# r9y9/deepvoice3_pytorch

Hardware: NVIDIA H100
Metric: mel-frames/sec training step (B=16,T_mel=800) (higher is better)
Workload: dtype f32 via split 16-bit pairs (fp16 pairs forward, bf16 pairs for gradients; 3 wgmma passes per product, fp32 accumulate)

## Files before the change

### deepvoice3_pytorch_b200/csrc/tc_gemm.cu

```cuda
#include "tc_common.cuh"
#include "../../include/dv3b200.h"

namespace dv3 {

using namespace tc;

constexpr int TC_CONV_THREADS = 512;
constexpr int TC_PRODUCER_REGS = 24;
constexpr int TC_CONSUMER_REGS = 176;
constexpr int TC_EPILOGUE_REGS = 136;
static_assert(TC_PRODUCER_REGS <= 65536 / TC_CONV_THREADS && TC_CONSUMER_REGS >= 65536 / TC_CONV_THREADS &&
              TC_EPILOGUE_REGS >= 65536 / TC_CONV_THREADS, "setmaxnreg direction of each warpgroup");
static_assert(128 * TC_PRODUCER_REGS + 256 * TC_CONSUMER_REGS + 128 * TC_EPILOGUE_REGS <= 65536, "register file");
constexpr int MAX_TAPS_TC = 8;
constexpr int SMEM_LIMIT = 232448;
constexpr int RING_RESERVE = 32768;

template <int STAGE_BYTES, int TILE_COLS, int RESERVE>
struct RingCfg {
    static constexpr int STAGE = STAGE_BYTES;
    static constexpr int NCOLS = TILE_COLS;
    static constexpr int ACC_PITCH = NCOLS + 1;
    static constexpr int ACC_TILE = 128 * ACC_PITCH * 4;
    static constexpr int STAGES_RAW = (SMEM_LIMIT - 2048 - RESERVE - ACC_TILE) / STAGE;
    static constexpr int STAGES = STAGES_RAW > 6 ? 6 : STAGES_RAW;
    static constexpr int SMEM = STAGES * STAGE + ACC_TILE + 1024 + 512;
};

enum { TC_GATED = 0, TC_CONV = 1 };

struct TcMaps { CUtensorMap a[2]; CUtensorMap b[2]; };

struct TcParams {
    int T;
    int Nc;
    int rows_per_tap;
    int k, kb_n;
    int tap_off[MAX_TAPS_TC];
    const float* bias; const float* spk; const float* res;
    float* y; float* save_a; float* save_s;
    int gate_mode, residual;
    float* out; const float* e1; const float* e2; float alpha; int addmode, relu;
    float p_drop; const unsigned long long* seed_ptr; uint32_t salt;
    float gmain;
    int operand_bf16;
};

template <int BK> struct SwizzleOf;
template <> struct SwizzleOf<64> { static constexpr uint32_t layout = WG_SW128, sbo = 1024; };
template <> struct SwizzleOf<32> { static constexpr uint32_t layout = WG_SW64, sbo = 512; };

template <int BK>
__device__ __forceinline__ uint64_t make_desc(uint32_t saddr) {
    return make_wgmma_desc(saddr, 16, SwizzleOf<BK>::sbo, SwizzleOf<BK>::layout);
}

template <int NBOX, int BK, int BR, int NPL = 2>
using TcCfg = RingCfg<NPL * (128 + NBOX * BR) * BK * 2, BR * NBOX, RING_RESERVE>;
static_assert(TcCfg<2, 32, 64>::STAGES == 4, "gated forward: 4-stage ring");
static_assert(TcCfg<1, 32, 128>::STAGES == 4, "128-column conv: 4-stage ring");
static_assert(TcCfg<1, 64, 64>::STAGES == 3, "64-column conv at BK = 64: 3-stage ring");
static_assert(TcCfg<1, 32, 64>::STAGES == 6, "64-column conv at BK = 32: 6-stage ring");
static_assert(TcCfg<2, 64, 64, 1>::STAGES == 4, "single-pass gated forward: 4-stage ring");
static_assert(TcCfg<1, 64, 128, 1>::STAGES == 4, "single-pass 128-column conv at BK = 64: 4-stage ring");
static_assert(TcCfg<1, 32, 128, 1>::STAGES == 6, "single-pass 128-column conv at BK = 32: 6-stage ring");
static_assert(TcCfg<1, 64, 64, 1>::STAGES == 6, "single-pass 64-column conv at BK = 64: 6-stage ring");
static_assert(TcCfg<1, 32, 64, 1>::STAGES == 6, "single-pass 64-column conv at BK = 32: 6-stage ring");

template <int BR>
__device__ __forceinline__ void epilogue_gated(const TcParams& p, const float* arow, uint64_t* acc_empty, int a_row0,
                                               int a_z, int b_row0) {
    const int t = a_row0 + (threadIdx.x & 127), b = a_z, C = p.Nc;
    const bool tv = t < p.T;
    const float* __restrict__ bias = p.bias;
    const float* __restrict__ res = p.res;
    const float* __restrict__ spk = p.spk;
    float* __restrict__ yo = p.y;
    float* __restrict__ ao = p.save_a;
    float* __restrict__ so = p.save_s;
    const bool need_res = (p.gate_mode != 0) || p.residual;
    const size_t base = ((size_t)b * C + b_row0) * p.T + (tv ? t : 0);
#pragma unroll
    for (int c32 = 0; c32 < BR; c32 += 32) {
        float rr[32], sp[32];
        if (tv) {
            const size_t cb = base + (size_t)c32 * p.T;
#pragma unroll
            for (int i = 0; i < 32; ++i) rr[i] = need_res ? __ldg(&res[cb + (size_t)i * p.T]) : 0.f;
            if (spk) {
#pragma unroll
                for (int i = 0; i < 32; ++i) sp[i] = __ldg(&spk[cb + (size_t)i * p.T]);
            }
#pragma unroll
            for (int i = 0; i < 32; ++i) {
                const int c = b_row0 + c32 + i;
                const size_t idx = cb + (size_t)i * p.T;
                float va = arow[c32 + i];
                if (spk) va += sp[i];
                const float a = va + __ldg(&bias[c]);
                const float s = sigmoidf_(arow[BR + c32 + i] + __ldg(&bias[C + c]));
                float y;
                if (p.gate_mode == 0) {
                    y = a * s;
                    if (p.residual) y = (y + rr[i]) * 0.70710678118654752f;
                } else {
                    y = s * a + (1.f - s) * rr[i];
                }
                yo[idx] = y;
                if (ao) ao[idx] = a;
                if (so) so[idx] = s;
            }
        }
        if (c32 + 32 == BR) mbar_arrive(acc_empty);
    }
}

template <int NCOLS>
__device__ __forceinline__ void epilogue_conv(const TcParams& p, const float* arow, uint64_t* acc_empty, int a_row0,
                                              int a_z, int b_row0) {
    const int t = a_row0 + (threadIdx.x & 127), b = a_z;
    const bool tv = t < p.T;
    const DropCfg drop = make_drop(p.p_drop, p.seed_ptr, p.salt);
    const float* __restrict__ bias = p.bias;
    const float* __restrict__ e1 = p.e1;
    const float* __restrict__ e2 = p.e2;
    float* __restrict__ out = p.out;
#pragma unroll 1
    for (int c32 = 0; c32 < NCOLS; c32 += 32) {
        float v[32], x2[32];
        const int n0 = b_row0 + c32;
        const size_t cb = ((size_t)b * p.Nc + n0) * p.T + (tv ? t : 0);
        if (tv) {
#pragma unroll
            for (int i = 0; i < 32; ++i) {
                const bool ok = n0 + i < p.Nc;
                v[i] = (p.addmode != 0 && ok) ? __ldg(&e1[cb + (size_t)i * p.T]) : 0.f;
                x2[i] = (p.addmode == 2 && ok) ? __ldg(&e2[cb + (size_t)i * p.T]) : 0.f;
            }
#pragma unroll
            for (int i = 0; i < 32; ++i) {
                const int n = n0 + i;
                if (n < p.Nc) {
                    const size_t idx = cb + (size_t)i * p.T;
                    float g = arow[c32 + i] * drop_scale(drop, (uint32_t)idx);
                    if (bias) g += __ldg(&bias[n]);
                    if (p.addmode == 1) g += p.alpha * v[i];
                    else if (p.addmode == 2) g += v[i] * (1.f - x2[i]);
                    if (p.relu) g = fmaxf(g, 0.f);
                    out[idx] = g;
                }
            }
        }
        if (c32 + 32 == NCOLS) mbar_arrive(acc_empty);
    }
}

template <class Cfg, int NPL, class Decode, class Load, class Mma, class Gmain, class Epilogue>
__device__ __forceinline__ void tc_pipeline(const TcMaps& maps, int num_units, Decode decode, Load load, Mma mma,
                                            Gmain gmain, Epilogue epilogue) {
    static_assert(NPL == 1 || NPL == 2, "one or two operand planes");
    static_assert(Cfg::NCOLS <= 128, "main + cross accumulators must fit in the registers of a consumer thread");
    static_assert(Cfg::STAGES >= 2, "pipeline needs at least two stages");
    constexpr int STAGE = Cfg::STAGE, STAGES = Cfg::STAGES;
    constexpr int NR = Cfg::NCOLS / 2;
    pdl_trigger();
    extern __shared__ uint8_t smem_raw[];
    uint8_t* smem = reinterpret_cast<uint8_t*>((reinterpret_cast<uintptr_t>(smem_raw) + 1023) & ~(uintptr_t)1023);
    float* acc_tile = reinterpret_cast<float*>(smem + STAGES * STAGE);
    uint64_t* full = reinterpret_cast<uint64_t*>(smem + STAGES * STAGE + Cfg::ACC_TILE);
    uint64_t* empty = full + STAGES;
    uint64_t* acc_full = empty + STAGES;
    uint64_t* acc_empty = acc_full + 1;
    const int warp = threadIdx.x >> 5, lane = threadIdx.x & 31;

    if (threadIdx.x == 0) {
#pragma unroll
        for (int pl = 0; pl < NPL; ++pl) prefetch_tmap(&maps.a[pl]);
#pragma unroll
        for (int pl = 0; pl < NPL; ++pl) prefetch_tmap(&maps.b[pl]);
        for (int s = 0; s < STAGES; ++s) { mbar_init(&full[s], 1); mbar_init(&empty[s], 2); }
        mbar_init(acc_full, 256);
        mbar_init(acc_empty, 128);
        fence_barrier_init();
    }
    __syncthreads();
    pdl_wait();

    if (warp >= 12) {
        setmaxnreg_inc<TC_EPILOGUE_REGS>();
        int n = 0;
        for (int u = blockIdx.x; u < num_units; u += gridDim.x, ++n) {
            const auto w = decode(u);
            mbar_wait(acc_full, n & 1);
            epilogue(w, acc_tile, acc_empty);
        }
    } else if (warp >= 8) {
        setmaxnreg_dec<TC_PRODUCER_REGS>();
        if (warp == 8 && lane == 0) {
            int it = 0;
            for (int u = blockIdx.x; u < num_units; u += gridDim.x) {
                const auto w = decode(u);
                for (int kit = 0; kit < w.n_iters; ++kit, ++it) {
                    const int s = it % STAGES, ph = (it / STAGES) & 1;
                    mbar_wait(&empty[s], ph ^ 1);
                    mbar_arrive_expect_tx(&full[s], STAGE);
                    load(w, kit, smem + s * STAGE, &full[s]);
                }
            }
        }
    } else {
        setmaxnreg_inc<TC_CONSUMER_REGS>();
        const int wg = warp >> 2, wq = warp & 3;
        float acc[NR], xacc[NPL == 2 ? NR : 1];
        int it = 0, n = 0;
        for (int u = blockIdx.x; u < num_units; u += gridDim.x, ++n) {
            const auto w = decode(u);
#pragma unroll
            for (int i = 0; i < NR; ++i) {
                acc[i] = 0.f;
                if constexpr (NPL == 2) xacc[i] = 0.f;
            }
            for (int kit = 0; kit < w.n_iters; ++kit, ++it) {
                const int s = it % STAGES, ph = (it / STAGES) & 1;
                mbar_wait(&full[s], ph);
                wgmma_fence();
                mma(smem + s * STAGE, wg, acc, xacc);
                wgmma_commit();
                wgmma_wait<1>();
                if (kit > 0 && (threadIdx.x & 127) == 0) mbar_arrive(&empty[(it - 1) % STAGES]);
            }
            wgmma_wait<0>();
            if (w.n_iters > 0 && (threadIdx.x & 127) == 0) mbar_arrive(&empty[(it - 1) % STAGES]);
            const float gm = gmain(w);
            mbar_wait(acc_empty, (n & 1) ^ 1);
#pragma unroll
            for (int i = 0; i < NR; ++i) {
                float* dst = &acc_tile[(64 * wg + frag_row(i, wq, lane)) * Cfg::ACC_PITCH + frag_col(i, lane)];
                if constexpr (NPL == 2) *dst = fmaf(xacc[i], LO_INV, acc[i] * gm);
                else *dst = acc[i] * gm;
            }
            mbar_arrive(acc_full);
        }
    }
}

template <int MODE, int NBOX, int BR, int BK, bool BF16, int NPL>
__global__ void __launch_bounds__(TC_CONV_THREADS, 1)
tc_conv_kernel(const __grid_constant__ TcMaps maps, const __grid_constant__ TcParams p, int tiles_x, int tiles_y,
               int num_tiles) {
    using Cfg = TcCfg<NBOX, BK, BR, NPL>;
    constexpr int NCOLS = Cfg::NCOLS;
    constexpr int TILE = 128 * BK * 2, TILE_B = BR * BK * 2;
    constexpr int B_OFF = NPL * TILE;
    constexpr int A_HALF = 64 * BK * 2;
    const int n_iters = p.k * p.kb_n;

    struct Tile { int a_row0, a_z, b_row0, b_row1, n_iters; };
    auto decode = [&](int tile) {
        Tile w;
        const int ty = tile % tiles_y, r = tile / tiles_y;
        w.a_z = r / tiles_x;
        w.a_row0 = (r % tiles_x) * 128;
        if (MODE == TC_GATED) { w.b_row0 = ty * BR; w.b_row1 = p.Nc + ty * BR; }
        else { w.b_row0 = ty * BR * NBOX; w.b_row1 = w.b_row0 + BR; }
        w.n_iters = n_iters;
        return w;
    };
    auto load = [&](const Tile& w, int kit, uint8_t* st, uint64_t* bar) {
        const int j = kit / p.kb_n, kb = kit - j * p.kb_n;
        const int ax = kb * BK, ay = w.a_row0 + p.tap_off[j];
        const int by0 = j * p.rows_per_tap + w.b_row0, by1 = j * p.rows_per_tap + w.b_row1;
#pragma unroll
        for (int pl = 0; pl < NPL; ++pl) {
            tma_load_3d(st + pl * TILE, &maps.a[pl], bar, ax, ay, w.a_z);
            uint8_t* bdst = st + B_OFF + pl * NBOX * TILE_B;
            tma_load_3d(bdst, &maps.b[pl], bar, ax, by0, 0);
            if (NBOX == 2) tma_load_3d(bdst + TILE_B, &maps.b[pl], bar, ax, by1, 0);
        }
    };
    auto mma = [&](const uint8_t* st, int wg, float* acc, float* xacc) {
        const uint32_t sa = smem_u32(st) + wg * A_HALF, sb = smem_u32(st + B_OFF);
#pragma unroll
        for (int kk = 0; kk < BK / 16; ++kk) {
            const uint32_t ko = kk * 32;
            const uint64_t a0 = make_desc<BK>(sa + ko), b0 = make_desc<BK>(sb + ko);
            wgmma_mma<NCOLS, 0, 0>(BF16, acc, a0, b0, 1);
            if constexpr (NPL == 2) {
                const uint64_t a1 = make_desc<BK>(sa + TILE + ko), b1 = make_desc<BK>(sb + NBOX * TILE_B + ko);
                wgmma_mma<NCOLS, 0, 0>(BF16, xacc, a0, b1, 1);
                wgmma_mma<NCOLS, 0, 0>(BF16, xacc, a1, b0, 1);
            }
        }
    };
    auto gmain = [&](const Tile&) { return p.gmain; };
    auto epilogue = [&](const Tile& w, const float* acc_tile, uint64_t* acc_empty) {
        const float* arow = acc_tile + (threadIdx.x & 127) * Cfg::ACC_PITCH;
        if (MODE == TC_GATED) epilogue_gated<BR>(p, arow, acc_empty, w.a_row0, w.a_z, w.b_row0);
        else epilogue_conv<NCOLS>(p, arow, acc_empty, w.a_row0, w.a_z, w.b_row0);
    };
    tc_pipeline<Cfg, NPL>(maps, num_tiles, decode, load, mma, gmain, epilogue);
}

struct TcMnParams {
    int T, B, Mw, Nw, k;
    int tap_off[MAX_TAPS_TC];
    int nsplit, batches_per_split, kb_n;
    int tiles_n, tiles_m, num_units;
    float* dw; long long split_stride;
    int msplit; long long s_m, s_mh, s_n, s_j;
    float gcoef;
};

constexpr int WG_BOX = 64 * 32 * 2;
template <int NPL>
using WgCfg = RingCfg<NPL * 4 * WG_BOX, 128, 0>;
static_assert(WgCfg<2>::STAGES == 5, "two-plane weight gradient: 5-stage ring");
static_assert(WgCfg<1>::STAGES == 6, "single-pass weight gradient: 6-stage ring");
static_assert(WgCfg<2>::SMEM <= SMEM_LIMIT && WgCfg<1>::SMEM <= SMEM_LIMIT, "weight gradient shared memory");

template <int NPL>
__global__ void __launch_bounds__(TC_CONV_THREADS, 1)
tc_wgrad_mn_kernel(const __grid_constant__ TcMaps maps, const __grid_constant__ TcMnParams p) {
    using Cfg = WgCfg<NPL>;
    constexpr int A_PL = 2 * WG_BOX, B_PL = 2 * WG_BOX;
    constexpr uint32_t LBO = 4096, SBO = 1024;

    struct Unit { int m0, n0, j, s, b_beg, n_iters; };
    auto decode = [&](int u) {
        Unit w;
        w.n0 = (u % p.tiles_n) * 128;
        int r = u / p.tiles_n;
        w.m0 = (r % p.tiles_m) * 128;
        r /= p.tiles_m;
        w.j = r % p.k;
        w.s = r / p.k;
        w.b_beg = w.s * p.batches_per_split;
        const int b_end = min(p.B, w.b_beg + p.batches_per_split);
        w.n_iters = (b_end > w.b_beg ? b_end - w.b_beg : 0) * p.kb_n;
        return w;
    };
    auto load = [&](const Unit& w, int kit, uint8_t* st, uint64_t* bar) {
        const int bi = kit / p.kb_n, tc_ = kit - bi * p.kb_n;
        const int b = w.b_beg + bi, t0 = tc_ * 32;
#pragma unroll
        for (int pl = 0; pl < NPL; ++pl) {
#pragma unroll
            for (int h = 0; h < 2; ++h)
                tma_load_3d(st + pl * A_PL + h * WG_BOX, &maps.a[pl], bar, w.m0 + h * 64, t0, b);
#pragma unroll
            for (int q = 0; q < 2; ++q)
                tma_load_3d(st + NPL * A_PL + pl * B_PL + q * WG_BOX, &maps.b[pl], bar, w.n0 + q * 64,
                            t0 + p.tap_off[w.j], b);
        }
    };
    auto mma = [&](const uint8_t* st, int wg, float* acc, float* xacc) {
        const uint32_t sa = smem_u32(st);
#pragma unroll
        for (int kk = 0; kk < 2; ++kk) {
            const uint32_t ko = kk * 16 * 128;
            const uint64_t a0 = make_wgmma_desc(sa + wg * WG_BOX + ko, LBO, SBO, WG_SW128);
            const uint64_t b0 = make_wgmma_desc(sa + NPL * A_PL + ko, LBO, SBO, WG_SW128);
            wgmma_mma<128, 1, 1>(true, acc, a0, b0, 1);
            if constexpr (NPL == 2) {
                const uint64_t a1 = make_wgmma_desc(sa + A_PL + wg * WG_BOX + ko, LBO, SBO, WG_SW128);
                const uint64_t b1 = make_wgmma_desc(sa + 2 * A_PL + B_PL + ko, LBO, SBO, WG_SW128);
                wgmma_mma<128, 1, 1>(true, xacc, a0, b1, 1);
                wgmma_mma<128, 1, 1>(true, xacc, a1, b0, 1);
            }
        }
    };
    auto gmain = [&](const Unit& w) { return 1.f + p.gcoef * (float)(2 * w.n_iters); };
    auto epilogue = [&](const Unit& w, const float* acc_tile, uint64_t* acc_empty) {
        const int r = threadIdx.x & 127;
        float* __restrict__ out = p.dw + (size_t)w.s * p.split_stride + (size_t)w.j * p.s_j;
        const int rows = min(128, p.Mw - w.m0), cols = min(128, p.Nw - w.n0);
        if (p.s_n == 1) {
            if (r < cols) {
                float* __restrict__ o = out + w.n0 + r;
#pragma unroll 4
                for (int i = 0; i < rows; ++i) {
                    const int m = w.m0 + i;
                    o[(size_t)(m % p.msplit) * p.s_m + (size_t)(m / p.msplit) * p.s_mh] = acc_tile[i * Cfg::ACC_PITCH + r];
                }
            }
        } else if (r < rows) {
            const int m = w.m0 + r;
            float* __restrict__ o = out + (size_t)(m % p.msplit) * p.s_m + (size_t)(m / p.msplit) * p.s_mh +
                                    (size_t)w.n0 * p.s_n;
            const float* arow = acc_tile + r * Cfg::ACC_PITCH;
#pragma unroll 4
            for (int c = 0; c < cols; ++c) o[(size_t)c * p.s_n] = arow[c];
        }
        mbar_arrive(acc_empty);
    };
    tc_pipeline<Cfg, NPL>(maps, p.num_units, decode, load, mma, gmain, epilogue);
}

typedef CUresult (*EncodeTiledFn)(CUtensorMap*, CUtensorMapDataType, cuuint32_t, void*, const cuuint64_t*,
                                  const cuuint64_t*, const cuuint32_t*, const cuuint32_t*, CUtensorMapInterleave,
                                  CUtensorMapSwizzle, CUtensorMapL2promotion, CUtensorMapFloatOOBfill);

static EncodeTiledFn encode_fn() {
    static const EncodeTiledFn fn = [] {
        void* f = nullptr;
        cudaDriverEntryPointQueryResult qres;
        cudaError_t e = cudaGetDriverEntryPoint("cuTensorMapEncodeTiled", &f, cudaEnableDefault, &qres);
        return (e == cudaSuccess) ? (EncodeTiledFn)f : (EncodeTiledFn) nullptr;
    }();
    return fn;
}

int encode_tmap_bf16_3d(CUtensorMap* map, const void* base, uint64_t d0, uint64_t d1, uint64_t d2,
                        uint64_t stride1_bytes, uint64_t stride2_bytes, uint32_t box0, uint32_t box1) {
    const EncodeTiledFn enc = encode_fn();
    if (!enc) { set_error("cuTensorMapEncodeTiled entry point unavailable"); return 1; }
    cuuint64_t dims[3] = {d0, d1, d2};
    cuuint64_t strides[2] = {stride1_bytes, stride2_bytes};
    cuuint32_t box[3] = {box0, box1, 1};
    cuuint32_t estr[3] = {1, 1, 1};
    const CUtensorMapSwizzle sw = box0 * 2 == 128 ? CU_TENSOR_MAP_SWIZZLE_128B : CU_TENSOR_MAP_SWIZZLE_64B;
    CUresult r = enc(map, CU_TENSOR_MAP_DATA_TYPE_BFLOAT16, 3, const_cast<void*>(base), dims, strides, box, estr,
                     CU_TENSOR_MAP_INTERLEAVE_NONE, sw, CU_TENSOR_MAP_L2_PROMOTION_L2_256B,
                     CU_TENSOR_MAP_FLOAT_OOB_FILL_NONE);
    if (r != CUDA_SUCCESS) {
        set_error("cuTensorMapEncodeTiled failed (%d): dims=(%llu,%llu,%llu) strides=(%llu,%llu) box=(%u,%u)", (int)r,
                  (unsigned long long)d0, (unsigned long long)d1, (unsigned long long)d2,
                  (unsigned long long)stride1_bytes, (unsigned long long)stride2_bytes, box0, box1);
        return 1;
    }
    return 0;
}

template <typename K>
static int ensure_smem(K kern, int bytes, const char* what) {
    cudaError_t e = cudaFuncSetAttribute(kern, cudaFuncAttributeMaxDynamicSharedMemorySize, bytes);
    if (e != cudaSuccess) { set_error("%s: cannot set %d B dynamic smem: %s", what, bytes, cudaGetErrorString(e)); return 1; }
    return 0;
}

template <class Cfg, auto kern, typename... Args>
static int launch_persistent(int units, cudaStream_t st, const char* what, const Args&... args) {
    static const int configured = ensure_smem(kern, Cfg::SMEM, what);
    if (configured) return 1;
    const int sms = config().sms, grid = units < sms ? units : sms;
    cudaError_t e = launch_k(kern, dim3(grid), dim3(TC_CONV_THREADS), (size_t)Cfg::SMEM, st, args...);
    if (e != cudaSuccess) { set_error("%s: launch failed: %s", what, cudaGetErrorString(e)); return 1; }
    return check_launch(what);
}

template <int MODE, int NBOX, int BR, int BK, bool BF16, int NPL>
static int launch_conv_fmt(const TcMaps& maps, const TcParams& p, int tiles_x, int tiles_y, int batch, cudaStream_t st,
                           const char* what) {
    const int num_tiles = tiles_x * tiles_y * batch;
    return launch_persistent<TcCfg<NBOX, BK, BR, NPL>, tc_conv_kernel<MODE, NBOX, BR, BK, BF16, NPL>>(
        num_tiles, st, what, maps, p, tiles_x, tiles_y, num_tiles);
}

template <int MODE, int NBOX, int BR, int BK, int NPL = 2>
static int launch_conv(const TcMaps& maps, const TcParams& p, int tiles_x, int tiles_y, int batch, cudaStream_t st,
                       const char* what) {
    if (p.operand_bf16)
        return launch_conv_fmt<MODE, NBOX, BR, BK, true, NPL>(maps, p, tiles_x, tiles_y, batch, st, what);
    return launch_conv_fmt<MODE, NBOX, BR, BK, false, NPL>(maps, p, tiles_x, tiles_y, batch, st, what);
}

static void fill_taps_tc(int* tap_off, int k, int dilation, int causal, bool transpose) {
    const int padl = causal ? (k - 1) * dilation : (k - 1) / 2 * dilation;
    for (int j = 0; j < MAX_TAPS_TC; ++j)
        tap_off[j] = j < k ? (transpose ? (padl - j * dilation) : (j * dilation - padl)) : 0;
}

static inline const void* plane(const void* base, int pl, long long plane_elems) {
    return (const char*)base + (size_t)pl * plane_elems * 2;
}

}

using namespace dv3;

extern "C" {

int dv3_tc_supported(int B, int C, int T, int k) {
    return (C % 128 == 0) && T >= 1 && k >= 1 && k <= MAX_TAPS_TC && B >= 1 && B <= 65535;
}
int dv3_tc_conv_supported(int B, int Cin, int Cout, int T, int k) {
    return T >= 1 && k >= 1 && k <= MAX_TAPS_TC && B >= 1 && B <= 65535 && (k == 1 || Cout % 128 == 0) && Cin >= 8 &&
           Cout >= 1;
}

int dv3_tc_convblock_fwd(const void* xd, const void* w, int npl, const float* bias, const float* spk,
                         const float* res, float* y, float* save_a, float* save_s, int B, int C, int T, int k,
                         int dilation, int causal, int mode, int residual, const void* fuse, void* stream) {
    DV3_REQUIRE(dv3_tc_supported(B, C, T, k), "tc_convblock_fwd: unsupported shape B=%d C=%d T=%d k=%d", B, C, T, k);
    DV3_REQUIRE(npl == 1 || npl == 2, "tc_convblock_fwd: npl must be 1 or 2");
    DV3_REQUIRE(fuse == nullptr, "tc_convblock_fwd: fuse must be NULL");
    TcMaps maps;
    const int t_tiles = (T + 127) / 128;
    const int BK = npl == 2 ? 32 : 64;
    for (int pl = 0; pl < npl; ++pl) {
        if (encode_tmap_bf16_3d(&maps.a[pl], plane(xd, pl, (long long)B * T * C), C, T, B, (uint64_t)C * 2,
                                (uint64_t)T * C * 2, BK, 128)) return 1;
        if (encode_tmap_bf16_3d(&maps.b[pl], plane(w, pl, (long long)k * 2 * C * C), C, (uint64_t)k * 2 * C, 1,
                                (uint64_t)C * 2, (uint64_t)k * 2 * C * C * 2, BK, 64)) return 1;
    }
    TcParams p = {};
    p.T = T; p.Nc = C; p.rows_per_tap = 2 * C; p.k = k; p.kb_n = C / BK;
    fill_taps_tc(p.tap_off, k, dilation, causal, false);
    p.bias = bias; p.spk = spk; p.res = res; p.y = y; p.save_a = save_a; p.save_s = save_s;
    p.gate_mode = mode; p.residual = residual;
    p.gmain = 1.f + config().tc_gamma * (float)(p.k * p.kb_n * (BK / 16));
    cudaStream_t st = (cudaStream_t)stream;
    if (npl == 1)
        return launch_conv_fmt<TC_GATED, 2, 64, 64, false, 1>(maps, p, t_tiles, C / 64, B, st, "tc_convblock_fwd");
    return launch_conv_fmt<TC_GATED, 2, 64, 32, false, 2>(maps, p, t_tiles, C / 64, B, st, "tc_convblock_fwd");
}

int dv3_tc_conv(const void* a, const void* w, int npl, float* out, int B, int Kc, int Nc, int T, int k, int dilation,
                int causal, int transpose_taps, const float* bias, int relu, float p_drop,
                const unsigned long long* seed_ptr, unsigned salt, int addmode, const float* e1, const float* e2,
                float alpha, const void* fuse, void* stream) {
    DV3_REQUIRE(k >= 1 && k <= MAX_TAPS_TC && (k == 1 || Nc % 128 == 0) && B <= 65535,
                "tc_conv: unsupported shape B=%d Kc=%d Nc=%d T=%d k=%d", B, Kc, Nc, T, k);
    DV3_REQUIRE(npl == 1 || npl == 2, "tc_conv: npl must be 1 or 2");
    DV3_REQUIRE(fuse == nullptr, "tc_conv: fuse must be NULL");
    const int Kp = (Kc + 7) / 8 * 8;
    const int t_tiles = (T + 127) / 128;
    cudaStream_t st = (cudaStream_t)stream;
    const long long tiles128 = (long long)t_tiles * ((Nc + 127) / 128) * B;
    const bool narrow = Nc > 64 && (k == 1 || Nc % 64 == 0) && tiles128 < 100;
    const bool k64 = Kc % 64 == 0;
    const int bk = ((narrow || npl == 1) && k64) ? 64 : 32, br = narrow ? 64 : 128;
    TcMaps maps;
    for (int pl = 0; pl < npl; ++pl) {
        if (encode_tmap_bf16_3d(&maps.a[pl], plane(a, pl, (long long)B * T * Kp), Kc, T, B, (uint64_t)Kp * 2,
                                (uint64_t)T * Kp * 2, bk, 128)) return 1;
        if (encode_tmap_bf16_3d(&maps.b[pl], plane(w, pl, (long long)k * Nc * Kp), Kc, (uint64_t)k * Nc, 1,
                                (uint64_t)Kp * 2, (uint64_t)k * Nc * Kp * 2, bk, br)) return 1;
    }
    TcParams p = {};
    p.T = T; p.Nc = Nc; p.rows_per_tap = Nc; p.k = k; p.kb_n = (Kc + bk - 1) / bk;
    fill_taps_tc(p.tap_off, k, dilation, causal, transpose_taps != 0);
    p.out = out; p.bias = bias; p.relu = relu; p.e1 = e1; p.e2 = e2; p.alpha = alpha; p.addmode = addmode;
    p.p_drop = p_drop; p.seed_ptr = seed_ptr; p.salt = salt;
    p.gmain = 1.f + config().tc_gamma * (float)(p.k * p.kb_n * (bk / 16));
    p.operand_bf16 = transpose_taps ? 1 : 0;
    const int tiles_y = (Nc + br - 1) / br;
    if (npl == 1) {
        if (narrow) {
            if (k64) return launch_conv<TC_CONV, 1, 64, 64, 1>(maps, p, t_tiles, tiles_y, B, st, "tc_conv(64)");
            return launch_conv<TC_CONV, 1, 64, 32, 1>(maps, p, t_tiles, tiles_y, B, st, "tc_conv(64,bk32)");
        }
        if (k64) return launch_conv<TC_CONV, 1, 128, 64, 1>(maps, p, t_tiles, tiles_y, B, st, "tc_conv(128,bk64)");
        return launch_conv<TC_CONV, 1, 128, 32, 1>(maps, p, t_tiles, tiles_y, B, st, "tc_conv(128)");
    }
    if (narrow) {
        if (k64) return launch_conv<TC_CONV, 1, 64, 64>(maps, p, t_tiles, tiles_y, B, st, "tc_conv(64)");
        return launch_conv<TC_CONV, 1, 64, 32>(maps, p, t_tiles, tiles_y, B, st, "tc_conv(64,bk32)");
    }
    return launch_conv<TC_CONV, 1, 128, 32>(maps, p, t_tiles, tiles_y, B, st, "tc_conv(128)");
}

constexpr double WG_UNIT_ITERS = 25.0;
constexpr double WG_SLAB_BYTES_PER_ITER = 1.5e6;
int dv3_tc_wgrad_nsplit(int B, int Mw, int Nw, int T, int k) {
    const long long tk = (long long)((Mw + 127) / 128) * ((Nw + 127) / 128) * k;
    const long long kb_n = (T + 31) / 32, sms = config().sms;
    const double slab = (double)Mw * Nw * k * 8.0 / WG_SLAB_BYTES_PER_ITER;
    auto cost = [&](int ns) {
        const long long bps = (B + ns - 1) / ns, U = tk * ns, U_full = tk * (ns - 1), G = U < sms ? U : sms;
        const long long L = bps * kb_n, L_last = (B - (ns - 1) * bps) * kb_n;
        return (double)((U_full + G - 1) / G) * (double)(L - L_last) +
               (double)((U + G - 1) / G) * ((double)L_last + WG_UNIT_ITERS) + ns * slab;
    };
    double best = 0.0;
    for (int bps = B, prev = 0; bps >= 1; --bps) {
        const int ns = (B + bps - 1) / bps;
        if (ns != prev && (prev == 0 || cost(ns) < best)) best = cost(ns);
        prev = ns;
    }
    for (int bps = B, prev = 0; bps >= 1; --bps) {
        const int ns = (B + bps - 1) / bps;
        if (ns != prev && cost(ns) <= 1.03 * best) return ns;
        prev = ns;
    }
    return 1;
}

int dv3_tc_wgrad_mn_npl(const void* dy, const void* xd, int npl, float* dw_partials, long long split_stride, int B,
                        int Mw, int Nw, int T, int k, int dilation, int causal, int msplit, long long s_m,
                        long long s_mh, long long s_n, long long s_j, void* stream) {
    DV3_REQUIRE(k >= 1 && k <= MAX_TAPS_TC && B <= 65535, "tc_wgrad_mn: unsupported shape k=%d", k);
    DV3_REQUIRE(npl == 1 || npl == 2, "tc_wgrad_mn: npl must be 1 or 2");
    const int Mp = (Mw + 7) / 8 * 8, Np = (Nw + 7) / 8 * 8;
    TcMaps maps;
    for (int pl = 0; pl < npl; ++pl) {
        if (encode_tmap_bf16_3d(&maps.a[pl], plane(dy, pl, (long long)B * T * Mp), Mw, T, B, (uint64_t)Mp * 2,
                                (uint64_t)T * Mp * 2, 64, 32)) return 1;
        if (encode_tmap_bf16_3d(&maps.b[pl], plane(xd, pl, (long long)B * T * Np), Nw, T, B, (uint64_t)Np * 2,
                                (uint64_t)T * Np * 2, 64, 32)) return 1;
    }
    TcMnParams p = {};
    p.T = T; p.B = B; p.Mw = Mw; p.Nw = Nw; p.k = k; p.kb_n = (T + 31) / 32;
    fill_taps_tc(p.tap_off, k, dilation, causal, false);
    p.nsplit = dv3_tc_wgrad_nsplit(B, Mw, Nw, T, k);
    p.batches_per_split = (B + p.nsplit - 1) / p.nsplit;
    p.tiles_n = (Nw + 127) / 128; p.tiles_m = (Mw + 127) / 128;
    const long long units = (long long)p.tiles_n * p.tiles_m * k * p.nsplit;
    DV3_REQUIRE(units < (1ll << 31), "tc_wgrad_mn: %lld work units", units);
    p.num_units = (int)units;
    p.dw = dw_partials; p.split_stride = split_stride;
    p.msplit = msplit; p.s_m = s_m; p.s_mh = s_mh; p.s_n = s_n; p.s_j = s_j;
    p.gcoef = config().tc_gamma;
    cudaStream_t st = (cudaStream_t)stream;
    if (npl == 1)
        return launch_persistent<WgCfg<1>, tc_wgrad_mn_kernel<1>>(p.num_units, st, "tc_wgrad_mn", maps, p);
    return launch_persistent<WgCfg<2>, tc_wgrad_mn_kernel<2>>(p.num_units, st, "tc_wgrad_mn", maps, p);
}

int dv3_tc_wgrad_mn(const void* dy, const void* xd, float* dw_partials, long long split_stride, int B, int Mw,
                    int Nw, int T, int k, int dilation, int causal, int msplit, long long s_m, long long s_mh,
                    long long s_n, long long s_j, void* stream) {
    return dv3_tc_wgrad_mn_npl(dy, xd, 2, dw_partials, split_stride, B, Mw, Nw, T, k, dilation, causal, msplit, s_m,
                               s_mh, s_n, s_j, stream);
}

}
```

Baseline: 1.545 million.

## Load one shared activation window per K-block and reuse it across conv taps

For two-plane bf16 transposed-tap convolutions (the backward data gradient), the kernel now loads a single activation window covering all tap offsets once per K block into a double-buffered shared-memory slot. Each tap's wgmma reads that window at a shifted row offset instead of issuing a separate 128-row TMA load per tap. The loop order changes to kb-major with taps inner, and new mbarriers manage the window slots. The aim is to cut redundant global and L2 traffic for activations when k>1. In exchange the weight ring is capped at 4 stages to make room, and the window slots add synchronization.

```diff
diff --git a/deepvoice3_pytorch_b200/csrc/tc_gemm.cu b/deepvoice3_pytorch_b200/csrc/tc_gemm.cu
--- a/deepvoice3_pytorch_b200/csrc/tc_gemm.cu
+++ b/deepvoice3_pytorch_b200/csrc/tc_gemm.cu
@@ -1,3 +1,4 @@
+#include <type_traits>
 #include "tc_common.cuh"
 #include "../../include/dv3b200.h"
 
@@ -15,16 +16,19 @@
 constexpr int MAX_TAPS_TC = 8;
 constexpr int SMEM_LIMIT = 232448;
 constexpr int RING_RESERVE = 32768;
-
-template <int STAGE_BYTES, int TILE_COLS, int RESERVE>
+constexpr int WIN_ROWS_MAX = 256;
+
+template <int STAGE_BYTES, int TILE_COLS, int RESERVE, int WIN_SLOT = 0, int WIN_SLOTS = 0, int MAX_STAGES = 6>
 struct RingCfg {
     static constexpr int STAGE = STAGE_BYTES;
+    static constexpr int WSLOT = WIN_SLOT, WSLOTS = WIN_SLOTS;
+    static constexpr int WIN = WSLOT * WSLOTS;
     static constexpr int NCOLS = TILE_COLS;
     static constexpr int ACC_PITCH = NCOLS + 1;
     static constexpr int ACC_TILE = 128 * ACC_PITCH * 4;
-    static constexpr int STAGES_RAW = (SMEM_LIMIT - 2048 - RESERVE - ACC_TILE) / STAGE;
-    static constexpr int STAGES = STAGES_RAW > 6 ? 6 : STAGES_RAW;
-    static constexpr int SMEM = STAGES * STAGE + ACC_TILE + 1024 + 512;
+    static constexpr int STAGES_RAW = (SMEM_LIMIT - 2048 - RESERVE - WIN - ACC_TILE) / STAGE;
+    static constexpr int STAGES = STAGES_RAW > MAX_STAGES ? MAX_STAGES : STAGES_RAW;
+    static constexpr int SMEM = WIN + STAGES * STAGE + ACC_TILE + 1024 + 512;
 };
 
 enum { TC_GATED = 0, TC_CONV = 1 };
@@ -37,6 +41,8 @@
     int rows_per_tap;
     int k, kb_n;
     int tap_off[MAX_TAPS_TC];
+    int win_off, win_rows;
+    int win_shift[MAX_TAPS_TC];
     const float* bias; const float* spk; const float* res;
     float* y; float* save_a; float* save_s;
     int gate_mode, residual;
@@ -66,6 +72,12 @@
 static_assert(TcCfg<1, 32, 128, 1>::STAGES == 6, "single-pass 128-column conv at BK = 32: 6-stage ring");
 static_assert(TcCfg<1, 64, 64, 1>::STAGES == 6, "single-pass 64-column conv at BK = 64: 6-stage ring");
 static_assert(TcCfg<1, 32, 64, 1>::STAGES == 6, "single-pass 64-column conv at BK = 32: 6-stage ring");
+
+template <int NBOX, int BK, int BR, int NPL = 2>
+using TcWinCfg = RingCfg<NPL * NBOX * BR * BK * 2, BR * NBOX, 0, NPL * WIN_ROWS_MAX * BK * 2, 2, 4>;
+static_assert(TcWinCfg<1, 32, 128>::STAGES == 4 && TcWinCfg<1, 64, 64>::STAGES == 4 && TcWinCfg<1, 32, 64>::STAGES == 4,
+              "window path: 4-stage weight rings");
+static_assert(TcWinCfg<1, 64, 64>::SMEM <= SMEM_LIMIT, "window path shared memory");
 
 template <int BR>
 __device__ __forceinline__ void epilogue_gated(const TcParams& p, const float* arow, uint64_t* acc_empty, int a_row0,
@@ -155,22 +167,27 @@
     }
 }
 
-template <class Cfg, int NPL, class Decode, class Load, class Mma, class Gmain, class Epilogue>
+struct NoWindow {};
+template <class Cfg, int NPL, class Decode, class Load, class Mma, class Gmain, class Epilogue, class LoadWin = NoWindow>
 __device__ __forceinline__ void tc_pipeline(const TcMaps& maps, int num_units, Decode decode, Load load, Mma mma,
-                                            Gmain gmain, Epilogue epilogue) {
+                                            Gmain gmain, Epilogue epilogue, int taps = 1, uint32_t win_bytes = 0,
+                                            LoadWin load_win = {}) {
     static_assert(NPL == 1 || NPL == 2, "one or two operand planes");
     static_assert(Cfg::NCOLS <= 128, "main + cross accumulators must fit in the registers of a consumer thread");
     static_assert(Cfg::STAGES >= 2, "pipeline needs at least two stages");
-    constexpr int STAGE = Cfg::STAGE, STAGES = Cfg::STAGES;
+    constexpr int STAGE = Cfg::STAGE, STAGES = Cfg::STAGES, WSLOTS = Cfg::WSLOTS;
     constexpr int NR = Cfg::NCOLS / 2;
     pdl_trigger();
     extern __shared__ uint8_t smem_raw[];
-    uint8_t* smem = reinterpret_cast<uint8_t*>((reinterpret_cast<uintptr_t>(smem_raw) + 1023) & ~(uintptr_t)1023);
+    uint8_t* const wins = reinterpret_cast<uint8_t*>((reinterpret_cast<uintptr_t>(smem_raw) + 1023) & ~(uintptr_t)1023);
+    uint8_t* const smem = wins + Cfg::WIN;
     float* acc_tile = reinterpret_cast<float*>(smem + STAGES * STAGE);
     uint64_t* full = reinterpret_cast<uint64_t*>(smem + STAGES * STAGE + Cfg::ACC_TILE);
     uint64_t* empty = full + STAGES;
     uint64_t* acc_full = empty + STAGES;
     uint64_t* acc_empty = acc_full + 1;
+    uint64_t* wfull = acc_empty + 1;
+    uint64_t* wempty = wfull + WSLOTS;
     const int warp = threadIdx.x >> 5, lane = threadIdx.x & 31;
 
     if (threadIdx.x == 0) {
@@ -181,6 +198,7 @@
         for (int s = 0; s < STAGES; ++s) { mbar_init(&full[s], 1); mbar_init(&empty[s], 2); }
         mbar_init(acc_full, 256);
         mbar_init(acc_empty, 128);
+        for (int s = 0; s < WSLOTS; ++s) { mbar_init(&wfull[s], 1); mbar_init(&wempty[s], 2); }
         fence_barrier_init();
     }
     __syncthreads();
@@ -197,10 +215,20 @@
     } else if (warp >= 8) {
         setmaxnreg_dec<TC_PRODUCER_REGS>();
         if (warp == 8 && lane == 0) {
-            int it = 0;
+            int it = 0, wit = 0;
             for (int u = blockIdx.x; u < num_units; u += gridDim.x) {
                 const auto w = decode(u);
-                for (int kit = 0; kit < w.n_iters; ++kit, ++it) {
+                for (int kit = 0, j = 0; kit < w.n_iters; ++kit, ++it) {
+                    if constexpr (WSLOTS > 0) {
+                        if (j == 0) {
+                            const int ws = wit % WSLOTS;
+                            mbar_wait(&wempty[ws], ((wit / WSLOTS) & 1) ^ 1);
+                            mbar_arrive_expect_tx(&wfull[ws], win_bytes);
+                            load_win(w, kit, wins + ws * Cfg::WSLOT, &wfull[ws]);
+                            ++wit;
+                        }
+                        if (++j == taps) j = 0;
+                    }
                     const int s = it % STAGES, ph = (it / STAGES) & 1;
                     mbar_wait(&empty[s], ph ^ 1);
                     mbar_arrive_expect_tx(&full[s], STAGE);
@@ -212,7 +240,7 @@
         setmaxnreg_inc<TC_CONSUMER_REGS>();
         const int wg = warp >> 2, wq = warp & 3;
         float acc[NR], xacc[NPL == 2 ? NR : 1];
-        int it = 0, n = 0;
+        int it = 0, wit = 0, n = 0;
         for (int u = blockIdx.x; u < num_units; u += gridDim.x, ++n) {
             const auto w = decode(u);
 #pragma unroll
@@ -220,17 +248,28 @@
                 acc[i] = 0.f;
                 if constexpr (NPL == 2) xacc[i] = 0.f;
             }
-            for (int kit = 0; kit < w.n_iters; ++kit, ++it) {
+            for (int kit = 0, j = 0; kit < w.n_iters; ++kit, ++it) {
                 const int s = it % STAGES, ph = (it / STAGES) & 1;
+                if constexpr (WSLOTS > 0) {
+                    if (j == 0) mbar_wait(&wfull[wit % WSLOTS], (wit / WSLOTS) & 1);
+                }
                 mbar_wait(&full[s], ph);
                 wgmma_fence();
-                mma(smem + s * STAGE, wg, acc, xacc);
+                if constexpr (WSLOTS > 0) mma(smem + s * STAGE, wins + (wit % WSLOTS) * Cfg::WSLOT, j, wg, acc, xacc);
+                else mma(smem + s * STAGE, wg, acc, xacc);
                 wgmma_commit();
                 wgmma_wait<1>();
                 if (kit > 0 && (threadIdx.x & 127) == 0) mbar_arrive(&empty[(it - 1) % STAGES]);
+                if constexpr (WSLOTS > 0) {
+                    if (kit > 0 && j == 0 && (threadIdx.x & 127) == 0) mbar_arrive(&wempty[(wit + WSLOTS - 1) % WSLOTS]);
+                    if (++j == taps) { j = 0; ++wit; }
+                }
             }
             wgmma_wait<0>();
-            if (w.n_iters > 0 && (threadIdx.x & 127) == 0) mbar_arrive(&empty[(it - 1) % STAGES]);
+            if (w.n_iters > 0 && (threadIdx.x & 127) == 0) {
+                mbar_arrive(&empty[(it - 1) % STAGES]);
+                if constexpr (WSLOTS > 0) mbar_arrive(&wempty[(wit + WSLOTS - 1) % WSLOTS]);
+            }
             const float gm = gmain(w);
             mbar_wait(acc_empty, (n & 1) ^ 1);
 #pragma unroll
@@ -244,15 +283,15 @@
     }
 }
 
-template <int MODE, int NBOX, int BR, int BK, bool BF16, int NPL>
-__global__ void __launch_bounds__(TC_CONV_THREADS, 1)
-tc_conv_kernel(const __grid_constant__ TcMaps maps, const __grid_constant__ TcParams p, int tiles_x, int tiles_y,
-               int num_tiles) {
-    using Cfg = TcCfg<NBOX, BK, BR, NPL>;
+template <int MODE, int NBOX, int BR, int BK, bool BF16, int NPL, bool WIN>
+__device__ __forceinline__ void tc_conv_body(const TcMaps& maps, const TcParams& p, int tiles_x, int tiles_y,
+                                             int num_tiles) {
+    using Cfg = std::conditional_t<WIN, TcWinCfg<NBOX, BK, BR, NPL>, TcCfg<NBOX, BK, BR, NPL>>;
     constexpr int NCOLS = Cfg::NCOLS;
     constexpr int TILE = 128 * BK * 2, TILE_B = BR * BK * 2;
-    constexpr int B_OFF = NPL * TILE;
+    constexpr int B_OFF = WIN ? 0 : NPL * TILE;
     constexpr int A_HALF = 64 * BK * 2;
+    constexpr int ROW = BK * 2, WPLANE = WIN_ROWS_MAX * ROW;
     const int n_iters = p.k * p.kb_n;
 
     struct Tile { int a_row0, a_z, b_row0, b_row1, n_iters; };
@@ -267,12 +306,14 @@
         return w;
     };
     auto load = [&](const Tile& w, int kit, uint8_t* st, uint64_t* bar) {
-        const int j = kit / p.kb_n, kb = kit - j * p.kb_n;
+        int j, kb;
+        if constexpr (WIN) { kb = kit / p.k; j = kit - kb * p.k; }
+        else { j = kit / p.kb_n; kb = kit - j * p.kb_n; }
         const int ax = kb * BK, ay = w.a_row0 + p.tap_off[j];
         const int by0 = j * p.rows_per_tap + w.b_row0, by1 = j * p.rows_per_tap + w.b_row1;
 #pragma unroll
         for (int pl = 0; pl < NPL; ++pl) {
-            tma_load_3d(st + pl * TILE, &maps.a[pl], bar, ax, ay, w.a_z);
+            if constexpr (!WIN) tma_load_3d(st + pl * TILE, &maps.a[pl], bar, ax, ay, w.a_z);
             uint8_t* bdst = st + B_OFF + pl * NBOX * TILE_B;
             tma_load_3d(bdst, &maps.b[pl], bar, ax, by0, 0);
             if (NBOX == 2) tma_load_3d(bdst + TILE_B, &maps.b[pl], bar, ax, by1, 0);
@@ -292,13 +333,50 @@
             }
         }
     };
+    auto load_win = [&](const Tile& w, int kit, uint8_t* slot, uint64_t* bar) {
+        const int ax = kit / p.k * BK, ay = w.a_row0 + p.win_off;
+#pragma unroll
+        for (int pl = 0; pl < NPL; ++pl) tma_load_3d(slot + pl * WPLANE, &maps.a[pl], bar, ax, ay, w.a_z);
+    };
+    auto mma_win = [&](const uint8_t* st, const uint8_t* slot, int j, int wg, float* acc, float* xacc) {
+        const uint32_t sa = smem_u32(slot) + (64 * wg + p.win_shift[j]) * ROW, sb = smem_u32(st);
+#pragma unroll
+        for (int kk = 0; kk < BK / 16; ++kk) {
+            const uint32_t ko = kk * 32;
+            const uint64_t a0 = make_desc<BK>(sa + ko), b0 = make_desc<BK>(sb + ko);
+            wgmma_mma<NCOLS, 0, 0>(BF16, acc, a0, b0, 1);
+            if constexpr (NPL == 2) {
+                const uint64_t a1 = make_desc<BK>(sa + WPLANE + ko), b1 = make_desc<BK>(sb + NBOX * TILE_B + ko);
+                wgmma_mma<NCOLS, 0, 0>(BF16, xacc, a0, b1, 1);
+                wgmma_mma<NCOLS, 0, 0>(BF16, xacc, a1, b0, 1);
+            }
+        }
+    };
     auto gmain = [&](const Tile&) { return p.gmain; };
     auto epilogue = [&](const Tile& w, const float* acc_tile, uint64_t* acc_empty) {
         const float* arow = acc_tile + (threadIdx.x & 127) * Cfg::ACC_PITCH;
         if (MODE == TC_GATED) epilogue_gated<BR>(p, arow, acc_empty, w.a_row0, w.a_z, w.b_row0);
         else epilogue_conv<NCOLS>(p, arow, acc_empty, w.a_row0, w.a_z, w.b_row0);
     };
-    tc_pipeline<Cfg, NPL>(maps, num_tiles, decode, load, mma, gmain, epilogue);
+    if constexpr (WIN)
+        tc_pipeline<Cfg, NPL>(maps, num_tiles, decode, load, mma_win, gmain, epilogue, p.k,
+                              (uint32_t)(NPL * p.win_rows * ROW), load_win);
+    else
+        tc_pipeline<Cfg, NPL>(maps, num_tiles, decode, load, mma, gmain, epilogue);
+}
+
+template <int MODE, int NBOX, int BR, int BK, bool BF16, int NPL>
+__global__ void __launch_bounds__(TC_CONV_THREADS, 1)
+tc_conv_kernel(const __grid_constant__ TcMaps maps, const __grid_constant__ TcParams p, int tiles_x, int tiles_y,
+               int num_tiles) {
+    tc_conv_body<MODE, NBOX, BR, BK, BF16, NPL, false>(maps, p, tiles_x, tiles_y, num_tiles);
+}
+
+template <int MODE, int NBOX, int BR, int BK, bool BF16, int NPL>
+__global__ void __launch_bounds__(TC_CONV_THREADS, 1)
+tc_conv_window_kernel(const __grid_constant__ TcMaps maps, const __grid_constant__ TcParams p, int tiles_x,
+                      int tiles_y, int num_tiles) {
+    tc_conv_body<MODE, NBOX, BR, BK, BF16, NPL, true>(maps, p, tiles_x, tiles_y, num_tiles);
 }
 
 struct TcMnParams {
@@ -452,6 +530,11 @@
 static int launch_conv_fmt(const TcMaps& maps, const TcParams& p, int tiles_x, int tiles_y, int batch, cudaStream_t st,
                            const char* what) {
     const int num_tiles = tiles_x * tiles_y * batch;
+    if constexpr (MODE == TC_CONV && BF16 && NPL == 2) {
+        if (p.win_rows > 0)
+            return launch_persistent<TcWinCfg<NBOX, BK, BR, NPL>, tc_conv_window_kernel<MODE, NBOX, BR, BK, BF16, NPL>>(
+                num_tiles, st, what, maps, p, tiles_x, tiles_y, num_tiles);
+    }
     return launch_persistent<TcCfg<NBOX, BK, BR, NPL>, tc_conv_kernel<MODE, NBOX, BR, BK, BF16, NPL>>(
         num_tiles, st, what, maps, p, tiles_x, tiles_y, num_tiles);
 }
@@ -468,6 +551,17 @@
     const int padl = causal ? (k - 1) * dilation : (k - 1) / 2 * dilation;
     for (int j = 0; j < MAX_TAPS_TC; ++j)
         tap_off[j] = j < k ? (transpose ? (padl - j * dilation) : (j * dilation - padl)) : 0;
+}
+
+static int set_window(TcParams& p) {
+    int lo = p.tap_off[0], hi = p.tap_off[0];
+    for (int j = 1; j < p.k; ++j) { lo = min(lo, p.tap_off[j]); hi = max(hi, p.tap_off[j]); }
+    p.win_rows = 0;
+    if (p.k == 1 || 128 + hi - lo > WIN_ROWS_MAX) return 128;
+    p.win_off = lo;
+    p.win_rows = 128 + hi - lo;
+    for (int j = 0; j < p.k; ++j) p.win_shift[j] = p.tap_off[j] - lo;
+    return p.win_rows;
 }
 
 static inline const void* plane(const void* base, int pl, long long plane_elems) {
@@ -497,15 +591,15 @@
     TcMaps maps;
     const int t_tiles = (T + 127) / 128;
     const int BK = npl == 2 ? 32 : 64;
+    TcParams p = {};
+    p.T = T; p.Nc = C; p.rows_per_tap = 2 * C; p.k = k; p.kb_n = C / BK;
+    fill_taps_tc(p.tap_off, k, dilation, causal, false);
     for (int pl = 0; pl < npl; ++pl) {
         if (encode_tmap_bf16_3d(&maps.a[pl], plane(xd, pl, (long long)B * T * C), C, T, B, (uint64_t)C * 2,
                                 (uint64_t)T * C * 2, BK, 128)) return 1;
         if (encode_tmap_bf16_3d(&maps.b[pl], plane(w, pl, (long long)k * 2 * C * C), C, (uint64_t)k * 2 * C, 1,
                                 (uint64_t)C * 2, (uint64_t)k * 2 * C * C * 2, BK, 64)) return 1;
     }
-    TcParams p = {};
-    p.T = T; p.Nc = C; p.rows_per_tap = 2 * C; p.k = k; p.kb_n = C / BK;
-    fill_taps_tc(p.tap_off, k, dilation, causal, false);
     p.bias = bias; p.spk = spk; p.res = res; p.y = y; p.save_a = save_a; p.save_s = save_s;
     p.gate_mode = mode; p.residual = residual;
     p.gmain = 1.f + config().tc_gamma * (float)(p.k * p.kb_n * (BK / 16));
@@ -530,16 +624,17 @@
     const bool narrow = Nc > 64 && (k == 1 || Nc % 64 == 0) && tiles128 < 100;
     const bool k64 = Kc % 64 == 0;
     const int bk = ((narrow || npl == 1) && k64) ? 64 : 32, br = narrow ? 64 : 128;
+    TcParams p = {};
+    p.T = T; p.Nc = Nc; p.rows_per_tap = Nc; p.k = k; p.kb_n = (Kc + bk - 1) / bk;
+    fill_taps_tc(p.tap_off, k, dilation, causal, transpose_taps != 0);
+    const int a_rows = (transpose_taps && npl == 2) ? set_window(p) : 128;
     TcMaps maps;
     for (int pl = 0; pl < npl; ++pl) {
         if (encode_tmap_bf16_3d(&maps.a[pl], plane(a, pl, (long long)B * T * Kp), Kc, T, B, (uint64_t)Kp * 2,
-                                (uint64_t)T * Kp * 2, bk, 128)) return 1;
+                                (uint64_t)T * Kp * 2, bk, a_rows)) return 1;
         if (encode_tmap_bf16_3d(&maps.b[pl], plane(w, pl, (long long)k * Nc * Kp), Kc, (uint64_t)k * Nc, 1,
                                 (uint64_t)Kp * 2, (uint64_t)k * Nc * Kp * 2, bk, br)) return 1;
     }
-    TcParams p = {};
-    p.T = T; p.Nc = Nc; p.rows_per_tap = Nc; p.k = k; p.kb_n = (Kc + bk - 1) / bk;
-    fill_taps_tc(p.tap_off, k, dilation, causal, transpose_taps != 0);
     p.out = out; p.bias = bias; p.relu = relu; p.e1 = e1; p.e2 = e2; p.alpha = alpha; p.addmode = addmode;
     p.p_drop = p_drop; p.seed_ptr = seed_ptr; p.salt = salt;
     p.gmain = 1.f + config().tc_gamma * (float)(p.k * p.kb_n * (bk / 16));
```

After: 1.564 million (median of 6 runs). +1.2%, better.
